# 0411tony/Yue

Measured on AMD Instinct MI355X. Metric: BPR triplet-updates/sec at k=128 (S-round semantics, user rows sequential; the reference's exact sequential semantics: secondary.exact), higher is better.
Workload: dtype f32

## Files before the change

### yue_amd/csrc/bpr_device.hpp

```cpp
#pragma once
#include <hip/hip_runtime.h>
#include <stdint.h>

namespace yue {

constexpr int kNllSlots = 1024;
constexpr int kMaxAttempts = 64;

struct TrainArgs {
    float *P, *Q, *dP, *dQ;
    float *stage;
#ifdef YUE_STAMPS
    unsigned long long *stamps;
#endif
    const int32_t *ev_u, *ev_i;
    int32_t *ev_j;
    const int64_t *indptr;
    const int32_t *indices;
    double *nll_slots;
    int64_t m, n;
    int k;
    float ru, ri;
    double lr;
    uint64_t seed;
    uint32_t epoch;
    int32_t neg_lo, neg_range;
};

struct RoundArgs {
    int64_t e_begin, e_end;
    int64_t n_begin, n_end;
    unsigned long long *cnt_cur;
    unsigned long long *cnt_next;
    uint32_t *cntp_cur;
    uint32_t *cntp_next;
    uint32_t *tab_cur, *tab_next;
    int staged;
    int apply_p;
};

__device__ __forceinline__ uint64_t mix64(uint64_t z) {
    z ^= z >> 30; z *= 0xBF58476D1CE4E5B9ull;
    z ^= z >> 27; z *= 0x94D049BB133111EBull;
    z ^= z >> 31; return z;
}

__device__ __forceinline__ int32_t ctr_draw(uint64_t seed, uint32_t epoch, uint64_t e, uint32_t a, int32_t lo, int32_t n_range) {
    uint64_t z = mix64(seed + 0x9E3779B97F4A7C15ull * (e + 1));
    z = mix64(z ^ (0xD1B54A32D192ED03ull * (uint64_t)(epoch + 1) + 0x8CB92BA72F3D8DD7ull * (uint64_t)a));
    return lo + (int32_t)(((z >> 32) * (uint64_t)(uint32_t)n_range) >> 32);
}

__device__ __forceinline__ bool csr_contains(const int64_t *indptr, const int32_t *indices, int64_t row, int32_t x) {
    int64_t lo = indptr[row], hi = indptr[row + 1];
    while (lo < hi) {
        int64_t mid = (lo + hi) >> 1;
        int32_t v = indices[mid];
        if (v < x) lo = mid + 1; else if (v > x) hi = mid; else return true;
    }
    return false;
}

__device__ __forceinline__ int32_t sample_negative(const TrainArgs &a, int32_t u, int64_t e) {
    for (uint32_t t = 0; t < (uint32_t)kMaxAttempts; ++t) {
        int32_t c = ctr_draw(a.seed, a.epoch, (uint64_t)e, t, a.neg_lo, a.neg_range);
        if (!csr_contains(a.indptr, a.indices, u, c)) return c;
    }
    return -1;
}

__device__ __forceinline__ float rdlane(float v, int l) {
    return __builtin_bit_cast(float, __builtin_amdgcn_readlane(__builtin_bit_cast(int, v), l));
}

template <int CTRL>
__device__ __forceinline__ float dpp_mov(float v) {
    return __builtin_bit_cast(float, __builtin_amdgcn_update_dpp(0, __builtin_bit_cast(int, v), CTRL, 0xF, 0xF, true));
}

__device__ __forceinline__ float wave_sum(float v) {
    v = v + dpp_mov<0xB1>(v);
    v = v + dpp_mov<0x4E>(v);
    v = v + dpp_mov<0x141>(v);
    v = v + dpp_mov<0x140>(v);
    float w = v;
    asm volatile("s_nop 1\n\tv_permlane16_swap_b32 %0, %1\n\ts_nop 1" : "+v"(v), "+v"(w));
    v = v + w;
    return rdlane(v, 0) + rdlane(v, 32);
}

__device__ __forceinline__ double chain_exp(double y) {
    const double n = __builtin_rint(y * 1.4426950408889634074);
    double r = __builtin_fma(-n, 6.93147180369123816490e-01, y);
    r = __builtin_fma(-n, 1.90821492927058770002e-10, r);
    const double r2 = r * r;
    const double a0 = __builtin_fma(r, 1.0, 1.0), a1 = __builtin_fma(r, 1.0 / 6.0, 0.5), a2 = __builtin_fma(r, 1.0 / 120.0, 1.0 / 24.0),
                 a3 = __builtin_fma(r, 1.0 / 5040.0, 1.0 / 720.0), a4 = __builtin_fma(r, 1.0 / 362880.0, 1.0 / 40320.0),
                 a5 = __builtin_fma(r, 1.0 / 39916800.0, 1.0 / 3628800.0), a6 = __builtin_fma(r, 1.0 / 6227020800.0, 1.0 / 479001600.0);
    const double r4 = r2 * r2;
    const double b0 = __builtin_fma(a1, r2, a0), b1 = __builtin_fma(a3, r2, a2), b2 = __builtin_fma(a5, r2, a4);
    const double r8 = r4 * r4;
    const double c0 = __builtin_fma(b1, r4, b0), c1 = __builtin_fma(a6, r4, b2);
    return __builtin_ldexp(__builtin_fma(c1, r8, c0), (int)n);
}
__device__ __forceinline__ double chain_rcp(double d) {
    double y = __builtin_amdgcn_rcp(d);
    double e = __builtin_fma(-d, y, 1.0);
    y = __builtin_fma(e, y, y);
    e = __builtin_fma(-d, y, 1.0);
    y = __builtin_fma(e, y, y);
    e = __builtin_fma(-d, y, 1.0);
    y = __builtin_fma(e, y, y);
    const double r = __builtin_fma(-d, y, 1.0);
    const double y2 = __builtin_bit_cast(double, __builtin_bit_cast(long long, y) + (r > 0.0 ? 1ll : -1ll));
    const double r2 = __builtin_fma(-d, y2, 1.0);
    return __builtin_fabs(r2) < __builtin_fabs(r) ? y2 : y;
}

__device__ __forceinline__ double chain_sigmoid(float x) {
    const double xd = (double)x;
    if (__builtin_fabs(xd) <= 700.0) return chain_rcp(1.0 + chain_exp(-xd));
    return 1.0 / (1.0 + exp(-xd));
}
__device__ __forceinline__ float chain_coef_fast(float x, float lr) {
    return lr * __builtin_amdgcn_rcpf(1.0f + __builtin_amdgcn_exp2f(x * 1.44269502162933349609375f));
}

__device__ __forceinline__ float wave_sum_any(float v) {
    v = v + dpp_mov<0xB1>(v);
    v = v + dpp_mov<0x4E>(v);
    v = v + dpp_mov<0x141>(v);
    v = v + dpp_mov<0x140>(v);
    v = v + __builtin_bit_cast(float, __builtin_amdgcn_update_dpp(0, __builtin_bit_cast(int, v), 0x142, 0xA, 0xF, false));
    v = v + __builtin_bit_cast(float, __builtin_amdgcn_update_dpp(0, __builtin_bit_cast(int, v), 0x143, 0xC, 0xF, false));
    return rdlane(v, 63);
}

struct Elem { float p2, qi2, qj2; };
__device__ __forceinline__ Elem bpr_elem(float p, float qi, float qj, float c, float ru, float ri) {
    const float d = qi - qj;
    const float td = c * d;
    const float p1 = p + td;
    const float tq = c * p1;
    const float qi1 = qi + tq;
    const float qj1 = qj - tq;
    const float rp = ru * p1;
    const float ra = ri * qi1;
    const float rb = ri * qj1;
    Elem o;
    o.p2 = p1 - rp;
    o.qi2 = qi1 - ra;
    o.qj2 = qj1 - rb;
    return o;
}

#define YUE_BLOAD(rs, vo, so) __builtin_bit_cast(float, __builtin_amdgcn_raw_buffer_load_b32((rs), (vo), (so), 0))
// ... 20 lines not shown
```

### yue_amd/csrc/bpr_host.hip

```cpp
#include "host_common.hpp"

#include "train_kernels.hpp"
#include "round_kernels.hpp"

using yue_host::fail;
using yue_host::kr_of;
using yue_host::with_kr;
static_assert(yue::kNllSlots == yue_host::kNllSlotsHost && yue::kHeaderSlack == yue_host::kHeaderSlackHost &&
              yue::kMetaStageMax == (uint32_t)yue_host::kMetaStageMaxHost, "host_common.hpp mirrors these");

namespace {

yue::TrainArgs make_args(yue_ctx *c, double lr, double regU, double regI) {
    yue::TrainArgs a{};
    a.P = c->P.p; a.Q = c->Q.p; a.dP = c->dP.p; a.dQ = c->dQ.p;
    a.stage = c->Q.p ? c->Q.p + (size_t)c->n * c->k : nullptr;
    a.ev_u = c->ev_u.p; a.ev_i = c->ev_i.p; a.ev_j = c->ev_j.p;
    a.indptr = c->indptr.p; a.indices = c->indices.p;
    a.nll_slots = c->scal.p;
    a.m = c->m; a.n = c->n; a.k = c->k;
    a.lr = lr;
    a.ru = (float)(lr * regU);
    a.ri = (float)(lr * regI);
    a.neg_lo = 0; a.neg_range = (int32_t)c->n;
    return a;
}

void launch_level(yue_ctx *c, const yue::TrainArgs &a, int64_t e0, int64_t e1) {
    const int tpw = (int)std::min<int64_t>(64, std::max<int64_t>(1, (e1 - e0) / 4096));
    const int64_t waves = (e1 - e0 + tpw - 1) / tpw;
    const dim3 grid((unsigned)((waves + 3) / 4)), block(256);
    with_kr(c->k, [&](auto kr) { hipLaunchKernelGGL(yue::k_bpr_level<kr()>, grid, block, 0, c->stream, a, e0, e1, tpw); });
}

constexpr int kRoundInstances[][2] = {{1, 8}, {1, 16}, {2, 8}, {4, 4}, {1, 4}, {2, 4}, {1, 2}, {2, 2}};

constexpr int default_round_tpw(int kr, bool meta) { return kr == 4 ? 4 : kr == 2 ? 8 : meta ? 8 : 16; }

template <class F, size_t... I>
bool with_round_instance(int kr, int tpw, F &&f, std::index_sequence<I...>) {
    return ((kr == kRoundInstances[I][0] && tpw == kRoundInstances[I][1] &&
             (f(std::integral_constant<int, kRoundInstances[I][0]>{}, std::integral_constant<int, kRoundInstances[I][1]>{}), true)) || ...);
}
template <class F>
bool with_round_instance(int kr, int tpw, F &&f) {
    return with_round_instance(kr, tpw, f, std::make_index_sequence<sizeof kRoundInstances / sizeof kRoundInstances[0]>{});
}

int tpw_of(const yue_ctx *c, bool meta) { return c->opt_round_tpw ? c->opt_round_tpw : default_round_tpw(kr_of(c->k), meta); }

constexpr int64_t kMetaRangeMax = 37 * 1024;
constexpr int64_t kMetaRangesMax = 12;
constexpr int64_t kRoundGenerationsMax = 6;
constexpr double kRoundEventsPerItemRow = 4.0;

bool meta_bucketed(const yue_ctx *c) { return c->n > kMetaRangeMax * kMetaRangesMax || c->opt_round_bucket; }
bool meta_path_fits(const yue_ctx *c) { return c->opt_round_meta && c->n <= ((int64_t)yue::kBucketRangesMax << yue::kBucketShift); }

// ... 435 lines not shown
    const size_t mk = (size_t)c->m * c->k * sizeof(float), nk = (size_t)c->n * c->k * sizeof(float);
    if (mU) HIPCHK(hipMemcpy(mU, c->aU_m.p, mk, hipMemcpyDeviceToHost));
    if (vU) HIPCHK(hipMemcpy(vU, c->aU_v.p, mk, hipMemcpyDeviceToHost));
    if (mV) HIPCHK(hipMemcpy(mV, c->aV_m.p, nk, hipMemcpyDeviceToHost));
    if (vV) HIPCHK(hipMemcpy(vV, c->aV_v.p, nk, hipMemcpyDeviceToHost));
    return YUE_OK;
}

int yue_adam_step(yue_ctx *c, const int32_t *u, const int32_t *i, const int32_t *j, int64_t T, double lr, double reg, int64_t step, double *loss_out) {
    if (!c || !c->have_factors) return fail(YUE_ERR_ARG, "yue_adam_step: no factors uploaded");
    if (T <= 0 || !u || !i || !j || step < 1) return fail(YUE_ERR_ARG, "yue_adam_step: bad argument (T > 0, step >= 1)");
    HIPCHK(hipSetDevice(c->device));
    if (c->adam_m != c->m || c->adam_n != c->n || c->adam_k != c->k) { const int rc0 = yue_adam_reset(c); if (rc0) return rc0; }
    for (int64_t t = 0; t < T; ++t)
        if (u[t] < 0 || u[t] >= c->m || i[t] < 0 || i[t] >= c->n || j[t] < 0 || j[t] >= c->n) return fail(YUE_ERR_ARG, "yue_adam_step: triplet " + std::to_string(t) + " out of range");
    int rc = upload_triplets(c, u, i, j, T, true);
    if (rc) return rc;
    if ((rc = zero_scalars(c))) return rc;
    yue::MbArgs a{};
    a.U = c->P.p; a.V = c->Q.p; a.gU = c->dP.p; a.gV = c->dQ.p; a.k = c->k; a.u = c->xu.p; a.i = c->xi.p; a.j = c->xj.p; a.T = T;
    a.reg = (float)reg; a.loss_slots = c->scal.p;
    const dim3 grid((unsigned)(((T + 31) / 32 + 3) / 4));
    with_kr(c->k, [&](auto kr) { hipLaunchKernelGGL(yue::k_mb_grad<kr()>, grid, dim3(256), 0, c->stream, a); });
    if ((rc = yue_host::adam_apply(c, lr, step))) return rc;
    return read_scalars(c, loss_out, nullptr, nullptr);
}

int yue_sample_negatives(yue_ctx *c, uint64_t seed, uint32_t epoch, int32_t *j_out) {
    if (!c || !c->have_inter || !j_out) return fail(YUE_ERR_ARG, "yue_sample_negatives: no interactions uploaded");
    HIPCHK(hipSetDevice(c->device));
    yue::TrainArgs a = make_args(c, 0, 0, 0);
    a.seed = seed; a.epoch = epoch;
    if (c->E > 0) {
        hipLaunchKernelGGL(yue::k_sample, dim3((unsigned)((c->E + 255) / 256)), dim3(256), 0, c->stream, a, c->E);
        HIPCHK(hipGetLastError());
        HIPCHK(hipMemcpyAsync(j_out, c->ev_j.p, c->E * sizeof(int32_t), hipMemcpyDeviceToHost, c->stream));
    }
    HIPCHK(hipStreamSynchronize(c->stream));
    return YUE_OK;
}

int yue_sumsq(yue_ctx *c, double *sp, double *sq) {
    if (!c || !c->have_factors) return fail(YUE_ERR_ARG, "yue_sumsq: no factors uploaded");
    HIPCHK(hipSetDevice(c->device));
    int rc = sumsq_async(c);
    if (rc) return rc;
    double h[2];
    HIPCHK(hipMemcpyAsync(h, c->scal.p + yue::kNllSlots + 1, sizeof h, hipMemcpyDeviceToHost, c->stream));
    HIPCHK(hipStreamSynchronize(c->stream));
    if (sp) *sp = h[0];
    if (sq) *sq = h[1];
    return YUE_OK;
}

int yue_bpr_epoch(yue_ctx *c, uint64_t seed, uint32_t epoch, int64_t round_events, double lr, double regU, double regI,
                  double *nll_out, double *sumsqP_out, double *sumsqQ_out) {
    if (!c || !c->have_factors || !c->have_inter) return fail(YUE_ERR_ARG, "yue_bpr_epoch: upload factors and interactions first");
    if (round_events < 0) return fail(YUE_ERR_ARG, "yue_bpr_epoch: round_events must be positive (or 0 for the device's default)");
    HIPCHK(hipSetDevice(c->device));
    yue::TrainArgs a = make_args(c, lr, regU, regI);
    a.seed = seed + 0x632BE59BD9B4E019ull * (uint64_t)c->rank;
    a.epoch = epoch;
    int rc = zero_scalars(c);
    if (rc) return rc;
    const int64_t E = c->E;
    if (E > 0) hipLaunchKernelGGL(yue::k_sample, dim3((unsigned)((E + 255) / 256)), dim3(256), 0, c->stream, a, E);
    if (c->opt_epoch_exact) {
        if (yue_host::on_communicator(c) && c->nranks > 1) return fail(YUE_ERR_ARG, "yue_bpr_epoch: option epoch_exact runs on one GPU (the sequential order spans all item shards)");
        if ((rc = yue_host::chain_epoch(c, lr, regU, regI))) return rc;
        if ((rc = sumsq_async(c))) return rc;
        return read_scalars(c, nll_out, sumsqP_out, sumsqQ_out);
    }
    std::vector<int64_t> bounds;
    double tot[2] = {(double)E, (double)c->n};
    if (yue_host::on_communicator(c)) {
        if ((rc = yue_allreduce_f64(c, tot, 2))) return rc;
        if ((rc = zero_scalars(c))) return rc;
    }
    const double etot = tot[0];
    if (round_events == 0 && (rc = default_round_events(c, tot[1] / c->nranks, &round_events))) return rc;
    int64_t ub = 1, group = 1;
    if ((rc = yue_epoch_plan(c->m, c->k, round_events, etot, c->nranks, &ub, &group, nullptr))) return rc;
    if (!yue_host::on_communicator(c)) group = std::max<int64_t>(1, (c->m + ub - 1) / ub);
    else group = std::max<int64_t>(1, ((int64_t)c->opt_comm_group_mb << 20) / std::max<int64_t>(1, ub * c->k * 4));
    std::vector<int64_t> ublock;
    for (int64_t u0 = 0; u0 < c->m; u0 += ub) { ublock.push_back(u0); bounds.push_back(c->h_ev_ptr[(size_t)u0]); }
    ublock.push_back(c->m); bounds.push_back(E);
    const int64_t R = (int64_t)ublock.size() - 1;
    const bool seq_user = !yue_host::on_communicator(c) && c->opt_round_user_seq && meta_path_fits(c);
    if (seq_user) {
        HIPCHK(c->d_ev_ptr.resize((size_t)c->m + 1));
        if (!c->d_ev_ptr_valid) {
            HIPCHK(hipMemcpyAsync(c->d_ev_ptr.p, c->h_ev_ptr.data(), ((size_t)c->m + 1) * sizeof(int64_t), hipMemcpyHostToDevice, c->stream));
            c->d_ev_ptr_valid = true;
        }
        HIPCHK(c->margins.resize((size_t)std::max<int64_t>(E, 1)));
    }
    c->psq_in_rounds = seq_user && c->all_users_have_events && E > 0;
    if (c->psq_in_rounds) {
        HIPCHK(c->psq_slots.resize((size_t)yue::kNllSlots));
        HIPCHK(hipMemsetAsync(c->psq_slots.p, 0, (size_t)yue::kNllSlots * sizeof(double), c->stream));
    }
    c->last_round_user_seq = 0;
    auto after = [&](int64_t r) -> int {
        if (seq_user && !c->bigq) { c->last_round_user_seq = 1; return YUE_OK; }
        if ((r + 1) % group != 0 && r + 1 != R) return YUE_OK;
        const int64_t g_first = ublock[(size_t)(r - (r % group))], g_last = ublock[(size_t)r + 1];
        const int64_t first = g_first * c->k, count = (g_last - g_first) * c->k;
        const dim3 grid((unsigned)std::min<int64_t>(4096, (count + 255) / 256));
        if (!yue_host::on_communicator(c)) {
            hipLaunchKernelGGL(yue::k_apply_range, grid, dim3(256), 0, c->stream, c->P.p, c->dP.p, first, count);
            return YUE_OK;
        }
        HIPCHK(hipEventRecord(c->ev_rounds, c->stream));
        HIPCHK(hipStreamWaitEvent(c->comm_stream, c->ev_rounds, 0));
        c->comm_collectives += 1;
        c->comm_bytes += (double)count * sizeof(float);
        if (const int rcr = yue_host::reduce_user_block(c, first, count, c->comm_stream)) return rcr;
        hipLaunchKernelGGL(yue::k_apply_range, grid, dim3(256), 0, c->comm_stream, c->P.p, c->dP.p, first, count);
        return YUE_OK;
    };
    c->comm_collectives = 0; c->comm_bytes = 0.0; c->comm_wait_ms = 0.0;
    if ((rc = run_rounds(c, a, bounds, 0, after, meta_path_fits(c), seq_user ? &ublock : nullptr))) { reset_round_state(c); return rc; }
    if (c->last_round_user_seq && E > 0)
        hipLaunchKernelGGL(yue::k_loss_margins, dim3(2048), dim3(256), 0, c->stream, c->margins.p, c->ev_j.p, E, c->scal.p);
    const bool psq_done = c->psq_in_rounds && c->last_round_user_seq;
    c->psq_in_rounds = false;
    if (yue_host::on_communicator(c)) {
        HIPCHK(hipEventRecord(c->ev_t_rounds, c->stream));
        HIPCHK(hipEventRecord(c->ev_t_comm, c->comm_stream));
    }
    HIPCHK(hipEventRecord(c->ev_comm, c->comm_stream));
    HIPCHK(hipStreamWaitEvent(c->stream, c->ev_comm, 0));
    c->comm_compute_waits = 1;
    HIPCHK(hipGetLastError());
    if ((rc = sumsq_async(c, psq_done ? c->psq_slots.p : nullptr))) return rc;
    if ((rc = read_scalars(c, nll_out, sumsqP_out, sumsqQ_out))) return rc;
    if (yue_host::on_communicator(c)) {
        float ms = 0.f;
        HIPCHK(hipEventSynchronize(c->ev_t_comm));
        HIPCHK(hipEventElapsedTime(&ms, c->ev_t_rounds, c->ev_t_comm));
        c->comm_wait_ms = ms > 0.f ? ms : 0.0;
    }
    return YUE_OK;
}

int yue_epoch_plan(int64_t m, int k, int64_t round_events, double events_total, int nranks,
                   int64_t *user_block, int64_t *blocks_per_group, int64_t *n_blocks) {
    if (m <= 0 || k <= 0 || round_events <= 0 || nranks < 1 || !(events_total >= 0.0)) return fail(YUE_ERR_ARG, "yue_epoch_plan: bad argument");
    const double per_user = events_total / (double)nranks / (double)m;
    const int64_t ub = std::max<int64_t>(1, (int64_t)std::floor((double)round_events / std::max(per_user, 1e-9) + 0.5));
    if (user_block) *user_block = ub;
    if (blocks_per_group) *blocks_per_group = std::max<int64_t>(1, (8ll << 20) / std::max<int64_t>(1, ub * k * 4));
    if (n_blocks) *n_blocks = (m + ub - 1) / ub;
    return YUE_OK;
}

int yue_default_round_events(yue_ctx *c, int64_t *out) {
// ... 50 lines not shown
```

### yue_amd/csrc/chain_host.hip

```cpp
#include "host_common.hpp"

#include <rocprim/rocprim.hpp>

#include "chain_kernels.hpp"

using yue_host::fail;
using yue_host::kr_of;

namespace {

int bits_for(uint64_t values) { int b = 1; while ((1ull << b) < values) ++b; return b; }

int rank_in_stream(yue_ctx *c, DevBuf<uint32_t> &key, DevBuf<uint32_t> &val, int64_t count, uint32_t nkeys, uint32_t *ord_a, uint32_t *ord_b) {
    if (count == 0) return YUE_OK;
    HIPCHK(c->ch_key2.resize((size_t)count)); HIPCHK(c->ch_val2.resize((size_t)count)); HIPCHK(c->ch_seg.resize((size_t)nkeys + 1));
    rocprim::double_buffer<uint32_t> dk(key.p, c->ch_key2.p), dv(val.p, c->ch_val2.p);
    size_t tmp = 0;
    const unsigned end_bit = (unsigned)bits_for((uint64_t)nkeys + 1);
    HIPCHK(rocprim::radix_sort_pairs(nullptr, tmp, dk, dv, (size_t)count, 0u, end_bit, c->stream));
    HIPCHK(c->ch_tmp.resize(tmp + 16));
    HIPCHK(rocprim::radix_sort_pairs(c->ch_tmp.p, tmp, dk, dv, (size_t)count, 0u, end_bit, c->stream));
    const dim3 grid((unsigned)((count + 255) / 256));
    hipLaunchKernelGGL(yue::k_chain_seg, grid, dim3(256), 0, c->stream, dk.current(), count, nkeys, c->ch_seg.p);
    hipLaunchKernelGGL(yue::k_chain_ord, grid, dim3(256), 0, c->stream, dk.current(), dv.current(), count, nkeys, c->ch_seg.p, ord_a, ord_b);
// ... 90 lines not shown
    const int64_t blocks = grid.x;
    hipLaunchKernelGGL(yue::k_chain_unpack, dim3(2048), dim3(256), 0, c->stream, c->ch_Qv.p, c->Q.p, n, k);
    if (ord_u) hipLaunchKernelGGL(yue::k_chain_unpack, dim3(2048), dim3(256), 0, c->stream, c->ch_Pv.p, c->P.p, m, k);
    HIPCHK(hipGetLastError());
    unsigned long long ctl[4];
    HIPCHK(hipMemcpyAsync(ctl, c->ch_ctl.p, sizeof ctl, hipMemcpyDeviceToHost, c->stream));
    HIPCHK(hipStreamSynchronize(c->stream));
    const uint32_t st = (uint32_t)ctl[2];
#ifdef YUE_CHAIN_STATS
    {
        unsigned long long h[8];
        HIPCHK(hipMemcpy(h, c->ch_stats.p, sizeof h, hipMemcpyDeviceToHost));
        if (split)
            fprintf(stderr, "[chain3 stats] per triplet: wave C %.0f cycles of work + %.0f waiting for a packet; wave L %.0f cycles per step without a wait (%llu steps) and %.0f waiting for room in the ring; wave S %.0f cycles waiting for packets or answers (%llu triplets)\n",
                    h[1] ? (double)h[0] / h[1] : 0.0, h[1] ? (double)h[2] / h[1] : 0.0, h[4] ? (double)h[3] / h[4] : 0.0, h[4], h[1] ? (double)h[7] / h[1] : 0.0, h[6] ? (double)h[5] / h[6] : 0.0, h[6]);
        else
        fprintf(stderr, "[chain stats] steps without a wait: %llu, %.0f cycles each; steps that waited: %llu (%.2f %%), %.0f cycles each; per run outside the steps: %.0f cycles (%llu runs)\n",
                h[1], h[1] ? (double)h[0] / h[1] : 0.0, h[3], 100.0 * h[3] / (double)(h[1] + h[3] + 1e-9), h[3] ? (double)h[2] / h[3] : 0.0, h[5] ? (double)h[4] / h[5] : 0.0, h[5]);
    }
#endif
    c->chain_runs = R; c->chain_waves = (one_xcd ? c->chain_groups : blocks) * waves_per_block;
    { float ms = 0.0f; HIPCHK(hipEventElapsedTime(&ms, c->ev_chain0, c->ev_chain1)); c->chain_kernel_us = (int64_t)(1e3 * ms); }
    if (st) return fail(YUE_ERR_HIP, std::string("exact path: a wave gave up waiting for a row (") + ((st & 2u) ? "a row's version ran past a waiting touch" : "spin limit") +
                                    "): internal error, the factors on the device are not usable");
    return YUE_OK;
}

}

namespace yue_host {

int chain_epoch(yue_ctx *c, double lr, double regU, double regI) {
    if (c->E == 0) return YUE_OK;
    HIPCHK(c->d_ev_ptr.resize((size_t)c->m + 1));
    if (!c->d_ev_ptr_valid) {
        HIPCHK(hipMemcpyAsync(c->d_ev_ptr.p, c->h_ev_ptr.data(), ((size_t)c->m + 1) * sizeof(int64_t), hipMemcpyHostToDevice, c->stream));
        c->d_ev_ptr_valid = true;
    }
    return chain_launch(c, nullptr, c->ev_i.p, c->ev_j.p, c->E, c->d_ev_ptr.p, nullptr, nullptr, c->m, lr, regU, regI);
}

int chain_stream(yue_ctx *c, int64_t T, double lr, double regU, double regI) {
    if (T == 0) return YUE_OK;
    if (T >= (1ll << 31)) return fail(YUE_ERR_ARG, "exact path: at most 2^31 - 1 triplets per call");
    HIPCHK(c->ch_head.resize((size_t)T)); HIPCHK(c->ch_incl.resize((size_t)T));
    const dim3 tgrid((unsigned)((T + 255) / 256));
    hipLaunchKernelGGL(yue::k_chain_heads, tgrid, dim3(256), 0, c->stream, c->xu.p, T, c->ch_head.p);
    size_t tmp = 0;
    HIPCHK(rocprim::inclusive_scan(nullptr, tmp, c->ch_head.p, c->ch_incl.p, (size_t)T, rocprim::plus<uint32_t>(), c->stream));
    HIPCHK(c->ch_tmp.resize(tmp + 16));
    HIPCHK(rocprim::inclusive_scan(c->ch_tmp.p, tmp, c->ch_head.p, c->ch_incl.p, (size_t)T, rocprim::plus<uint32_t>(), c->stream));
    uint32_t R32 = 0;
    HIPCHK(hipMemcpyAsync(&R32, c->ch_incl.p + (T - 1), sizeof R32, hipMemcpyDeviceToHost, c->stream));
    HIPCHK(hipStreamSynchronize(c->stream));
    const int64_t R = R32;
    HIPCHK(c->ch_run_ptr.resize((size_t)R + 1)); HIPCHK(c->ch_run_u.resize((size_t)R)); HIPCHK(c->ch_ord_u.resize((size_t)R));
    HIPCHK(c->ch_rkey.resize((size_t)R)); HIPCHK(c->ch_rval.resize((size_t)R));
    hipLaunchKernelGGL(yue::k_chain_runs, tgrid, dim3(256), 0, c->stream, c->xu.p, c->ch_head.p, c->ch_incl.p, T, c->ch_run_ptr.p, c->ch_run_u.p, c->ch_rkey.p, c->ch_rval.p, (uint32_t)c->m);
    int rc = rank_in_stream(c, c->ch_rkey, c->ch_rval, R, (uint32_t)c->m, c->ch_ord_u.p, nullptr);
    if (rc) return rc;
    return chain_launch(c, c->xu.p, c->xi.p, c->xj.p, T, c->ch_run_ptr.p, c->ch_run_u.p, c->ch_ord_u.p, R, lr, regU, regI);
}

}
```

### yue_amd/csrc/core_host.hip

```cpp
#include "host_common.hpp"

namespace yue_host {
thread_local std::string g_err;
int fail(int code, const std::string &msg) { g_err = msg; return code; }
}
using yue_host::fail;
void yue_comm_release(yue_ctx *c);

extern "C" {

const char *yue_last_error(void) { return yue_host::g_err.c_str(); }
int yue_version(void) { return 1; }

int yue_ctx_create(int device, yue_ctx **out) {
    if (!out) return fail(YUE_ERR_ARG, "yue_ctx_create: out is NULL");
    int ndev = 0;
    HIPCHK(hipGetDeviceCount(&ndev));
    if (ndev <= 0) return fail(YUE_ERR_HIP, "no HIP device visible: libyue_hip needs an MI355X (no CPU fallback exists)");
    if (device < 0 || device >= ndev) return fail(YUE_ERR_ARG, "device ordinal out of range");
    HIPCHK(hipSetDevice(device));
    yue_ctx *c = new yue_ctx();
    c->device = device;
    const auto init = [c]() -> int {
        HIPCHK(hipStreamCreateWithFlags(&c->stream, hipStreamNonBlocking));
// ... 98 lines not shown
    return YUE_OK;
}

int yue_set_interactions(yue_ctx *c, const int64_t *indptr, const int32_t *indices, const int64_t *ev_ptr, const int32_t *ev_i) {
    if (!c || !indptr || !indices || !ev_ptr || !ev_i) return fail(YUE_ERR_ARG, "yue_set_interactions: null argument");
    if (!c->have_factors) return fail(YUE_ERR_ARG, "yue_set_interactions: call yue_set_factors first (m, n)");
    HIPCHK(hipSetDevice(c->device));
    const int64_t m = c->m, n = c->n;
    if (indptr[0] != 0 || ev_ptr[0] != 0) return fail(YUE_ERR_ARG, "yue_set_interactions: indptr[0] and ev_ptr[0] must be 0");
    for (int64_t u = 0; u < m; ++u) {
        if (indptr[u + 1] < indptr[u] || ev_ptr[u + 1] < ev_ptr[u]) return fail(YUE_ERR_ARG, "yue_set_interactions: offsets must be non-decreasing");
        for (int64_t t = indptr[u]; t < indptr[u + 1]; ++t) {
            if (indices[t] < 0 || indices[t] >= n) return fail(YUE_ERR_ARG, "yue_set_interactions: item id out of range");
            if (t > indptr[u] && indices[t] <= indices[t - 1]) return fail(YUE_ERR_ARG, "yue_set_interactions: rows must be sorted and unique");
        }
        if (indptr[u + 1] - indptr[u] >= n) return fail(YUE_ERR_ARG, "yue_set_interactions: a user listened to every item (the reference's sampler would never return, BPR.py:47)");
    }
    const int64_t nnz = indptr[m], E = ev_ptr[m];
    {
        int64_t prev = -1, max_gap = 0;
        for (int64_t u = 0; u < m; ++u) if (ev_ptr[u + 1] > ev_ptr[u]) { if (prev >= 0) max_gap = std::max(max_gap, u - prev); prev = u; }
        if (max_gap * c->k * 4 >= (1ll << 31)) return fail(YUE_ERR_ARG, "yue_set_interactions: more than 2 GiB of user-factor rows between two consecutive users with events");
    }
    std::vector<int32_t> evu((size_t)E);
    for (int64_t u = 0; u < m; ++u)
        for (int64_t e = ev_ptr[u]; e < ev_ptr[u + 1]; ++e) {
            if (ev_i[e] < 0 || ev_i[e] >= n) return fail(YUE_ERR_ARG, "yue_set_interactions: event item out of range");
            evu[(size_t)e] = (int32_t)u;
        }
    c->E = E; c->nnz = nnz;
    c->h_ev_ptr.assign(ev_ptr, ev_ptr + m + 1);
    c->all_users_have_events = true;
    for (int64_t u = 0; u < m; ++u) if (ev_ptr[u + 1] <= ev_ptr[u]) { c->all_users_have_events = false; break; }
    c->d_ev_ptr_valid = false;
    HIPCHK(c->indptr.resize(m + 1)); HIPCHK(c->indices.resize(std::max<int64_t>(nnz, 1)));
    HIPCHK(c->ev_u.resize((size_t)E + yue_host::kHeaderSlackHost)); HIPCHK(c->ev_i.resize((size_t)E + yue_host::kHeaderSlackHost)); HIPCHK(c->ev_j.resize((size_t)E + yue_host::kHeaderSlackHost));
    HIPCHK(hipMemcpyAsync(c->indptr.p, indptr, (m + 1) * sizeof(int64_t), hipMemcpyHostToDevice, c->stream));
    HIPCHK(hipMemcpyAsync(c->indices.p, indices, nnz * sizeof(int32_t), hipMemcpyHostToDevice, c->stream));
    HIPCHK(hipMemcpyAsync(c->ev_u.p, evu.data(), E * sizeof(int32_t), hipMemcpyHostToDevice, c->stream));
    HIPCHK(hipMemcpyAsync(c->ev_i.p, ev_i, E * sizeof(int32_t), hipMemcpyHostToDevice, c->stream));
    HIPCHK(hipStreamSynchronize(c->stream));
    c->have_inter = true;
    return YUE_OK;
}


}
```

### yue_amd/csrc/host_common.hpp

```cpp
#pragma once
#include "../../include/yue_hip.h"

#include <hip/hip_runtime.h>

#include <algorithm>
#include <cmath>
#include <cstdio>
#include <cstdlib>
#include <cstring>
#include <string>
#include <type_traits>
#include <vector>

struct ncclComm;
struct yue_wrmf;
struct yue_knn;
struct yue_expo;
struct yue_cof;
struct yue_cnet;
struct yue_s2v;
struct yue_lgcn;
struct yue_ipf;

namespace yue_host {
// ... 104 lines not shown
    int opt_round_bucket = 0;
    int opt_fold_blocks = 1536;
    int opt_round_user_seq = 1;
    int opt_round_fast = 1;
    int last_round_user_seq = 0;
    int opt_comm_group_mb = 8;
    int opt_round_cus_reserved = 0;
    int64_t comm_compute_waits = 0;
    int opt_round_meta = 1;
    int timing_stride = 0;
    std::vector<std::pair<hipEvent_t, hipEvent_t>> ev_pool;
    std::vector<int64_t> ev_triplets, ev_launches;
    size_t ev_used = 0;
    DevBuf<double> fP, fBi, f_coef, f_x, f_hist, f_scores, f_out_sc;
    DevBuf<float> fQ;
    DevBuf<int64_t> f_ptr;
    DevBuf<int32_t> f_items, f_negs, f_ids, f_flags;
    DevBuf<int64_t> f_uq_ptr, f_neg_ptr;
    DevBuf<int32_t> f_uq_items, f_loc_i, f_loc_j;
    DevBuf<float> f_wq, f_dQ;
    DevBuf<double> f_wp, f_wb, f_dP, f_dB;
    DevBuf<unsigned> f_cnt;
    int64_t fn = 0;
    int fk = 0;
    int opt_fism_inplace = 1;
    int opt_fism_lds = 1;
    DevBuf<uint32_t> ch_key, ch_val, ch_key2, ch_val2, ch_seg, ch_ord_i, ch_ord_j, ch_head, ch_incl, ch_ord_u, ch_rkey, ch_rval;
    DevBuf<int64_t> ch_run_ptr, d_ev_ptr;
    DevBuf<int32_t> ch_run_u;
    DevBuf<unsigned char> ch_tmp;
    DevBuf<unsigned> ch_Qv, ch_Pv;
    DevBuf<unsigned long long> ch_ctl;
    DevBuf<unsigned long long> ch_stats;
    bool d_ev_ptr_valid = false;
    int opt_epoch_exact = 0;
    int opt_replay_levels = 0;
    int opt_chain_split = -1;
    int opt_chain_ring = 0;
    int opt_chain_xcd = 0;
    int opt_chain_fast = 0;
    int opt_chain_waves = 0;
    int64_t opt_chain_spin = 0;
    int64_t chain_runs = 0, chain_waves = 0, chain_groups = 0, chain_kernel_us = 0, replay_levels = 0;
    hipEvent_t ev_chain0 = nullptr, ev_chain1 = nullptr;
    ncclComm *comm = nullptr;
    int rank = 0, nranks = 1;
    hipStream_t comm_stream = nullptr;
    hipEvent_t ev_rounds = nullptr, ev_comm = nullptr;
    hipEvent_t ev_t_rounds = nullptr, ev_t_comm = nullptr;
    int (*seam_reduce)(void *host, int64_t count, int dtype, void *user) = nullptr;
    void *seam_user = nullptr;
    std::vector<float> seam_buf;
    int64_t comm_collectives = 0;
    double comm_bytes = 0.0, comm_wait_ms = 0.0;
    int comm_version = 0, comm_nranks_reported = 0;
    hipEvent_t ev_scan0 = nullptr, ev_scan1 = nullptr;
    yue_wrmf *wrmf = nullptr;
    yue_knn *knn = nullptr;
    yue_ipf *ipf = nullptr;
    yue_expo *expo = nullptr;
    yue_cof *cof = nullptr;
    yue_cnet *cnet = nullptr;
    yue_s2v *s2v = nullptr;
    yue_lgcn *lgcn = nullptr;
    int64_t opt_lgcn_hub = 1024;
    int64_t lgcn_hubs = 0, lgcn_parts = 0;
    int64_t lgcn_ns[4] = {0, 0, 0, 0};
// ... 45 lines not shown
```

### yue_amd/csrc/round_kernels.hpp

```cpp
#pragma once
#include "train_kernels.hpp"

#ifdef YUE_ABL_NO_HOT
#define YUE_M_HOT(val, rs, vo, so) asm volatile("" :: "v"(val))
#else
#define YUE_M_HOT(val, rs, vo, so) YUE_BATOMIC(val, rs, vo, so)
#endif
#ifdef YUE_ABL_NO_DP
#define YUE_M_DP(val, rs, vo, so) asm volatile("" :: "v"(val))
#else
#define YUE_M_DP(val, rs, vo, so) YUE_BATOMIC(val, rs, vo, so)
#endif

#define YUE_BLOAD_NT(rs, vo, so) __builtin_bit_cast(float, __builtin_amdgcn_raw_buffer_load_b32((rs), (vo), (so), 2))
#if defined(YUE_EXP_LOAD_CACHED)
#define YUE_M_LOAD_J(rs, vo, so) YUE_BLOAD(rs, vo, so)
#define YUE_M_LOAD_I(rs, vo, so) YUE_BLOAD(rs, vo, so)
#elif defined(YUE_EXP_LOAD_NT)
#define YUE_M_LOAD_J(rs, vo, so) YUE_BLOAD_NT(rs, vo, so)
#define YUE_M_LOAD_I(rs, vo, so) YUE_BLOAD_NT(rs, vo, so)
#else
#define YUE_M_LOAD_J(rs, vo, so) YUE_BLOAD_NT(rs, vo, so)
#define YUE_M_LOAD_I(rs, vo, so) YUE_BLOAD(rs, vo, so)
#endif
// ... 399 lines not shown
    const int64_t wave = (int64_t)blockIdx.x * 4 + __builtin_amdgcn_readfirstlane((int)(threadIdx.x >> 6));
    const int64_t u = ra.u_begin + wave;
    if (u >= ra.u_end) return;
    const int64_t e0 = ra.ev_ptr[u], e1 = ra.ev_ptr[u + 1];
    if (e1 <= e0) return;
    const unsigned k = (unsigned)a.k;
    const unsigned row_bytes = k * 4u;
    unsigned vo[KR];
#pragma unroll
    for (int r = 0; r < KR; ++r) { const unsigned e = 64u * r + lane; vo[r] = e < k ? e * 4u : kOobOffset; }
    const uint64_t qbytes = (uint64_t)a.n * row_bytes;
    const int qrec = (int)(qbytes < 0x7fffffffull ? qbytes : 0x7fffffffull);
    const unsigned stage0 = (unsigned)a.n * row_bytes;
    const uint64_t qsbytes = qbytes + (ra.staged ? 2ull * (uint64_t)(ra.e_end - ra.e_begin) * row_bytes : 0ull);
    const int qsrec = (int)(qsbytes < 0x7fffffffull ? qsbytes : 0x7fffffffull);
    const auto rsQ = __builtin_amdgcn_make_buffer_rsrc(a.Q, 0, qsrec, kRsrcFlags);
    const auto rsdQ = __builtin_amdgcn_make_buffer_rsrc(a.dQ, 0, qrec, kRsrcFlags);
    float *prow = a.P + (uint64_t)u * k;
    float p[KR];
#pragma unroll
    for (int r = 0; r < KR; ++r) { const unsigned e = 64u * r + lane; p[r] = e < k ? prow[e] : 0.0f; }
    const float lrf = (float)a.lr;
    const unsigned len = (unsigned)(e1 - e0 < 0x7fffffff ? e1 - e0 : 0x7fffffff);
    for (unsigned seg = 0; seg < len; seg += 64u) {
        int hI, hJ;
        uint32_t hMI, hMJ;
        {
            const bool ex = seg + (unsigned)lane < len;
            const int64_t e = e0 + seg + (ex ? lane : 0);
            hI = evi[e]; hJ = evj[e]; hMI = mti[e]; hMJ = mtj[e];
            if (!ex) { hI = 0; hJ = -1; hMI = 0u; hMJ = 0u; }
        }
        const unsigned seg_len = len - seg < 64u ? len - seg : 64u;
        float xs = 0.0f;
        auto gather = [&](float (&qi)[KR], float (&qj)[KR], unsigned t) {
            const int ti = __builtin_amdgcn_readlane(hI, t), tj = __builtin_amdgcn_readlane(hJ, t);
            const unsigned oi = (unsigned)ti * row_bytes, oj = (unsigned)(tj < 0 ? 0 : tj) * row_bytes;
#pragma unroll
            for (int r = 0; r < KR; ++r) { qi[r] = YUE_M_LOAD_I(rsQ, vo[r], oi); qj[r] = YUE_M_LOAD_J(rsQ, vo[r], oj); }
        };
        auto step = [&](const float (&qi)[KR], const float (&qj)[KR], unsigned t) {
            const int tj = __builtin_amdgcn_readlane(hJ, t);
            if (tj < 0) return;
            const int ti = __builtin_amdgcn_readlane(hI, t);
            const uint32_t mi = (uint32_t)__builtin_amdgcn_readlane((int)hMI, t), mj = (uint32_t)__builtin_amdgcn_readlane((int)hMJ, t);
            float ai = 0.0f, aj = 0.0f;
#pragma unroll
            for (int r = 0; r < KR; ++r) { const float a1 = p[r] * qi[r]; ai = ai + a1; const float a2 = p[r] * qj[r]; aj = aj + a2; }
            const float x = wave_sum(ai) - wave_sum(aj);
            const float c = FAST ? chain_coef_fast(x, lrf) : (float)(a.lr * (1.0 - chain_sigmoid(x)));
            xs = (unsigned)lane == t ? x : xs;
            const unsigned cli = meta_kind(mi), clj = meta_kind(mj);
            const bool uniq_i = cli == kMetaUnique, uniq_j = clj == kMetaUnique;
            const bool full_i = uniq_i || meta_first(mi), full_j = uniq_j || meta_first(mj);
            const unsigned oi = (unsigned)ti * row_bytes, oj = (unsigned)tj * row_bytes;
            const unsigned wi = uniq_i ? oi : stage0 + meta_slot(mi) * row_bytes;
            const unsigned wj = uniq_j ? oj : stage0 + meta_slot(mj) * row_bytes;
            Elem o[KR];
#pragma unroll
            for (int r = 0; r < KR; ++r) { o[r] = bpr_elem(p[r], qi[r], qj[r], c, a.ru, a.ri); p[r] = o[r].p2; }
            if (cli != kMetaHot) {
#pragma unroll
                for (int r = 0; r < KR; ++r) YUE_BSTORE(full_i ? o[r].qi2 : o[r].qi2 - qi[r], rsQ, vo[r], wi);
            } else {
#pragma unroll
                for (int r = 0; r < KR; ++r) YUE_M_HOT(o[r].qi2 - qi[r], rsdQ, vo[r], oi);
            }
            if (clj != kMetaHot) {
#pragma unroll
                for (int r = 0; r < KR; ++r) YUE_BSTORE(full_j ? o[r].qj2 : o[r].qj2 - qj[r], rsQ, vo[r], wj);
            } else {
#pragma unroll
                for (int r = 0; r < KR; ++r) YUE_M_HOT(o[r].qj2 - qj[r], rsdQ, vo[r], oj);
            }
        };
        constexpr int D = KR == 1 ? 8 : 4;
        float qi[D][KR], qj[D][KR];
#pragma unroll
        for (int s_ = 0; s_ < D; ++s_) gather(qi[s_], qj[s_], (unsigned)s_);
        for (unsigned t = 0; t < seg_len; t += D) {
#pragma unroll
            for (int s_ = 0; s_ < D; ++s_) {
                step(qi[s_], qj[s_], t + s_);
                gather(qi[s_], qj[s_], (t + s_ + D) & 63u);
            }
        }
        if ((unsigned)lane < seg_len) ra.margins[e0 + seg + lane] = xs;
    }
#pragma unroll
    for (int r = 0; r < KR; ++r) { const unsigned e = 64u * r + lane; if (e < k) prow[e] = p[r]; }
    if (ra.psq_slots) {
        double s = 0.0;
#pragma unroll
        for (int r = 0; r < KR; ++r) { const unsigned e = 64u * r + lane; const float sq = p[r] * p[r]; if (e < k) s += (double)sq; }
#pragma unroll
        for (int off = 1; off < 64; off <<= 1) s += __shfl_xor(s, off);
        if (lane == 0) atomicAdd(ra.psq_slots + (u & (kNllSlots - 1)), s);
    }
}

__global__ void __launch_bounds__(256) k_loss_margins(const float *__restrict__ x, const int32_t *__restrict__ evj, int64_t E, double *nll_slots) {
    double nl = 0.0;
    const int64_t stride = (int64_t)gridDim.x * blockDim.x;
    for (int64_t e = (int64_t)blockIdx.x * blockDim.x + threadIdx.x; e < E; e += stride)
        if (evj[e] >= 0) nl += -log(chain_sigmoid(x[e]));
#pragma unroll
    for (int off = 1; off < 64; off <<= 1) nl += __shfl_xor(nl, off);
    if ((threadIdx.x & 63) == 0 && nl != 0.0) atomicAdd(nll_slots + ((blockIdx.x * 4 + (threadIdx.x >> 6)) & (kNllSlots - 1)), nl);
}

struct FoldArgs {
    const uint2 *fold;
    const unsigned long long *round_rows;
    float *Q, *dQ;
    const float *stage;
    int k;
    uint32_t capacity;
};

template <int KR, int EPG>
__device__ __forceinline__ void fold_group(const FoldArgs &f, int lane, unsigned k, uint32_t nact, const uint2 (&ent)[4]) {
    float st[EPG][4][KR];
    unsigned el[KR];
    bool big = false;
#pragma unroll
    for (int r = 0; r < KR; ++r) el[r] = min(64u * r + lane, k - 1u);
#pragma unroll
    for (int sl = 0; sl < EPG; ++sl) {
        if ((uint32_t)sl >= nact) continue;
        const uint32_t c = fold_count(ent[sl].y);
        const bool hot = c == 0u;
        const float *src = hot ? f.dQ + (uint64_t)ent[sl].x * k : f.stage + (uint64_t)fold_block(ent[sl].y) * k;
#pragma unroll
        for (int r = 0; r < KR; ++r) st[sl][0][r] = YUE_FOLD_LD(src + el[r]);
        if (hot) {
            const float *row = f.Q + (uint64_t)ent[sl].x * k;
#pragma unroll
            for (int r = 0; r < KR; ++r) st[sl][1][r] = YUE_FOLD_LDROW(row + el[r]);
// ... 95 lines not shown
```

### yue_amd/csrc/train_kernels.hpp

```cpp
#pragma once
#include "bpr_device.hpp"

namespace yue {

__global__ void __launch_bounds__(256) k_sample(TrainArgs a, int64_t E) {
    int64_t e = (int64_t)blockIdx.x * blockDim.x + threadIdx.x;
    if (e < E) a.ev_j[e] = sample_negative(a, a.ev_u[e], e);
}

template <int KR>
__global__ void __launch_bounds__(256) k_bpr_level(TrainArgs a, int64_t e_begin, int64_t e_end, int tpw) {
    const int lane = threadIdx.x & 63;
    const int64_t wave = (int64_t)blockIdx.x * (blockDim.x >> 6) + (threadIdx.x >> 6);
    const int64_t base = e_begin + wave * tpw;
    if (base >= e_end) return;
    const int cnt = (int)((e_end - base) < (int64_t)tpw ? (e_end - base) : (int64_t)tpw);
    int u = 0, i = 0, j = 0;
    if (lane < cnt) { u = a.ev_u[base + lane]; i = a.ev_i[base + lane]; j = a.ev_j[base + lane]; }
    const int k = a.k;
    double nll = 0.0;
    for (int t = 0; t < cnt; ++t) {
        const int64_t tu = __builtin_amdgcn_readlane(u, t);
        const int64_t ti = __builtin_amdgcn_readlane(i, t);
        const int64_t tj = __builtin_amdgcn_readlane(j, t);
        float p[KR], qi[KR], qj[KR];
#pragma unroll
        for (int r = 0; r < KR; ++r) {
            const int e = 64 * r + lane;
            p[r] = e < k ? a.P[tu * k + e] : 0.0f;
            qi[r] = e < k ? a.Q[ti * k + e] : 0.0f;
            qj[r] = e < k ? a.Q[tj * k + e] : 0.0f;
        }
        float ai = 0.0f, aj = 0.0f;
#pragma unroll
        for (int r = 0; r < KR; ++r) { const float a1 = p[r] * qi[r]; ai = ai + a1; const float a2 = p[r] * qj[r]; aj = aj + a2; }
        const float x = wave_sum(ai) - wave_sum(aj);
        const double s = 1.0 / (1.0 + exp(-(double)x));
        const float c = (float)(a.lr * (1.0 - s));
        nll += -log(s);
#pragma unroll
// ... 472 lines not shown
```

Measured before the change: 1.794 billion.

## Sample negatives per user wave with lane-resident rows; vectorize loss kernel

Adds a user-major negative sampler. Each wave owns a user, keeps short CSR rows (up to 64 items) in lanes and tests membership with a ds_bpermute binary search instead of a global-memory binary search per candidate. It prefetches the next user's pointers and row, and falls back to the old per-event kernel when users have few events. The loss kernel now reads margins as float4, takes one log of the product of four sigmoid inverses, and drops the ev_j check by seeding skipped margins with a large sentinel. The ev_ptr upload moves to setup. This trades a small numeric change in the loss sum (product-then-log, sentinel adds a tiny nonzero term) for less memory traffic.

```diff
diff --git a/yue_amd/csrc/bpr_device.hpp b/yue_amd/csrc/bpr_device.hpp
--- a/yue_amd/csrc/bpr_device.hpp
+++ b/yue_amd/csrc/bpr_device.hpp
@@ -45,20 +45,35 @@
     z ^= z >> 31; return z;
 }
 
-__device__ __forceinline__ int32_t ctr_draw(uint64_t seed, uint32_t epoch, uint64_t e, uint32_t a, int32_t lo, int32_t n_range) {
-    uint64_t z = mix64(seed + 0x9E3779B97F4A7C15ull * (e + 1));
-    z = mix64(z ^ (0xD1B54A32D192ED03ull * (uint64_t)(epoch + 1) + 0x8CB92BA72F3D8DD7ull * (uint64_t)a));
+__device__ __forceinline__ uint64_t ctr_draw_event(uint64_t seed, uint64_t e) { return mix64(seed + 0x9E3779B97F4A7C15ull * (e + 1)); }
+__device__ __forceinline__ int32_t ctr_draw_attempt(uint64_t ze, uint32_t epoch, uint32_t a, int32_t lo, int32_t n_range) {
+    const uint64_t z = mix64(ze ^ (0xD1B54A32D192ED03ull * (uint64_t)(epoch + 1) + 0x8CB92BA72F3D8DD7ull * (uint64_t)a));
     return lo + (int32_t)(((z >> 32) * (uint64_t)(uint32_t)n_range) >> 32);
 }
+__device__ __forceinline__ int32_t ctr_draw(uint64_t seed, uint32_t epoch, uint64_t e, uint32_t a, int32_t lo, int32_t n_range) {
+    return ctr_draw_attempt(ctr_draw_event(seed, e), epoch, a, lo, n_range);
+}
 
-__device__ __forceinline__ bool csr_contains(const int64_t *indptr, const int32_t *indices, int64_t row, int32_t x) {
-    int64_t lo = indptr[row], hi = indptr[row + 1];
+__device__ __forceinline__ bool sorted_contains(const int32_t *indices, int64_t lo, int64_t hi, int32_t x) {
     while (lo < hi) {
         int64_t mid = (lo + hi) >> 1;
         int32_t v = indices[mid];
         if (v < x) lo = mid + 1; else if (v > x) hi = mid; else return true;
     }
     return false;
+}
+__device__ __forceinline__ bool csr_contains(const int64_t *indptr, const int32_t *indices, int64_t row, int32_t x) {
+    return sorted_contains(indices, indptr[row], indptr[row + 1], x);
+}
+
+__device__ __forceinline__ bool lanes_contain(int32_t row, int32_t x) {
+    int pos = 0;
+#pragma unroll
+    for (int step = 32; step >= 1; step >>= 1) {
+        const int32_t v = __builtin_amdgcn_ds_bpermute((pos + step - 1) << 2, row);
+        pos += v < x ? step : 0;
+    }
+    return __builtin_amdgcn_ds_bpermute(pos << 2, row) == x;
 }
 
 __device__ __forceinline__ int32_t sample_negative(const TrainArgs &a, int32_t u, int64_t e) {
@@ -122,6 +137,11 @@
     if (__builtin_fabs(xd) <= 700.0) return chain_rcp(1.0 + chain_exp(-xd));
     return 1.0 / (1.0 + exp(-xd));
 }
+__device__ __forceinline__ double chain_inv_sigmoid(float x) {
+    const double xd = (double)x;
+    return 1.0 + (__builtin_fabs(xd) <= 700.0 ? chain_exp(-xd) : exp(-xd));
+}
+constexpr float kMarginNoNegative = 128.0f;
 __device__ __forceinline__ float chain_coef_fast(float x, float lr) {
     return lr * __builtin_amdgcn_rcpf(1.0f + __builtin_amdgcn_exp2f(x * 1.44269502162933349609375f));
 }
diff --git a/yue_amd/csrc/bpr_host.hip b/yue_amd/csrc/bpr_host.hip
--- a/yue_amd/csrc/bpr_host.hip
+++ b/yue_amd/csrc/bpr_host.hip
@@ -24,6 +24,15 @@
     a.ri = (float)(lr * regI);
     a.neg_lo = 0; a.neg_range = (int32_t)c->n;
     return a;
+}
+
+void launch_sample(yue_ctx *c, const yue::TrainArgs &a) {
+    if (c->E >= (int64_t)yue::kSampleWaveEvents * c->m) {
+        const dim3 grid((unsigned)std::min<int64_t>(yue::kSampleBlocksMax, (c->m + 3) / 4));
+        hipLaunchKernelGGL(yue::k_sample, grid, dim3(256), 0, c->stream, a, c->d_ev_ptr.p, c->indptr.p, c->indices.p, c->ev_j.p);
+    } else {
+        hipLaunchKernelGGL(yue::k_sample_events, dim3((unsigned)((c->E + 255) / 256)), dim3(256), 0, c->stream, a, c->E);
+    }
 }
 
 void launch_level(yue_ctx *c, const yue::TrainArgs &a, int64_t e0, int64_t e1) {
@@ -525,7 +534,7 @@
     yue::TrainArgs a = make_args(c, 0, 0, 0);
     a.seed = seed; a.epoch = epoch;
     if (c->E > 0) {
-        hipLaunchKernelGGL(yue::k_sample, dim3((unsigned)((c->E + 255) / 256)), dim3(256), 0, c->stream, a, c->E);
+        launch_sample(c, a);
         HIPCHK(hipGetLastError());
         HIPCHK(hipMemcpyAsync(j_out, c->ev_j.p, c->E * sizeof(int32_t), hipMemcpyDeviceToHost, c->stream));
     }
@@ -557,7 +566,7 @@
     int rc = zero_scalars(c);
     if (rc) return rc;
     const int64_t E = c->E;
-    if (E > 0) hipLaunchKernelGGL(yue::k_sample, dim3((unsigned)((E + 255) / 256)), dim3(256), 0, c->stream, a, E);
+    if (E > 0) launch_sample(c, a);
     if (c->opt_epoch_exact) {
         if (yue_host::on_communicator(c) && c->nranks > 1) return fail(YUE_ERR_ARG, "yue_bpr_epoch: option epoch_exact runs on one GPU (the sequential order spans all item shards)");
         if ((rc = yue_host::chain_epoch(c, lr, regU, regI))) return rc;
@@ -581,14 +590,7 @@
     ublock.push_back(c->m); bounds.push_back(E);
     const int64_t R = (int64_t)ublock.size() - 1;
     const bool seq_user = !yue_host::on_communicator(c) && c->opt_round_user_seq && meta_path_fits(c);
-    if (seq_user) {
-        HIPCHK(c->d_ev_ptr.resize((size_t)c->m + 1));
-        if (!c->d_ev_ptr_valid) {
-            HIPCHK(hipMemcpyAsync(c->d_ev_ptr.p, c->h_ev_ptr.data(), ((size_t)c->m + 1) * sizeof(int64_t), hipMemcpyHostToDevice, c->stream));
-            c->d_ev_ptr_valid = true;
-        }
-        HIPCHK(c->margins.resize((size_t)std::max<int64_t>(E, 1)));
-    }
+    if (seq_user) HIPCHK(c->margins.resize((size_t)std::max<int64_t>(E, 1)));
     c->psq_in_rounds = seq_user && c->all_users_have_events && E > 0;
     if (c->psq_in_rounds) {
         HIPCHK(c->psq_slots.resize((size_t)yue::kNllSlots));
@@ -616,7 +618,7 @@
     c->comm_collectives = 0; c->comm_bytes = 0.0; c->comm_wait_ms = 0.0;
     if ((rc = run_rounds(c, a, bounds, 0, after, meta_path_fits(c), seq_user ? &ublock : nullptr))) { reset_round_state(c); return rc; }
     if (c->last_round_user_seq && E > 0)
-        hipLaunchKernelGGL(yue::k_loss_margins, dim3(2048), dim3(256), 0, c->stream, c->margins.p, c->ev_j.p, E, c->scal.p);
+        hipLaunchKernelGGL(yue::k_loss_margins, dim3(2048), dim3(256), 0, c->stream, c->margins.p, E, c->scal.p);
     const bool psq_done = c->psq_in_rounds && c->last_round_user_seq;
     c->psq_in_rounds = false;
     if (yue_host::on_communicator(c)) {
diff --git a/yue_amd/csrc/chain_host.hip b/yue_amd/csrc/chain_host.hip
--- a/yue_amd/csrc/chain_host.hip
+++ b/yue_amd/csrc/chain_host.hip
@@ -146,11 +146,6 @@
 
 int chain_epoch(yue_ctx *c, double lr, double regU, double regI) {
     if (c->E == 0) return YUE_OK;
-    HIPCHK(c->d_ev_ptr.resize((size_t)c->m + 1));
-    if (!c->d_ev_ptr_valid) {
-        HIPCHK(hipMemcpyAsync(c->d_ev_ptr.p, c->h_ev_ptr.data(), ((size_t)c->m + 1) * sizeof(int64_t), hipMemcpyHostToDevice, c->stream));
-        c->d_ev_ptr_valid = true;
-    }
     return chain_launch(c, nullptr, c->ev_i.p, c->ev_j.p, c->E, c->d_ev_ptr.p, nullptr, nullptr, c->m, lr, regU, regI);
 }
 
diff --git a/yue_amd/csrc/core_host.hip b/yue_amd/csrc/core_host.hip
--- a/yue_amd/csrc/core_host.hip
+++ b/yue_amd/csrc/core_host.hip
@@ -154,11 +154,11 @@
     c->h_ev_ptr.assign(ev_ptr, ev_ptr + m + 1);
     c->all_users_have_events = true;
     for (int64_t u = 0; u < m; ++u) if (ev_ptr[u + 1] <= ev_ptr[u]) { c->all_users_have_events = false; break; }
-    c->d_ev_ptr_valid = false;
-    HIPCHK(c->indptr.resize(m + 1)); HIPCHK(c->indices.resize(std::max<int64_t>(nnz, 1)));
+    HIPCHK(c->indptr.resize(m + 1)); HIPCHK(c->indices.resize(std::max<int64_t>(nnz, 1))); HIPCHK(c->d_ev_ptr.resize((size_t)m + 1));
     HIPCHK(c->ev_u.resize((size_t)E + yue_host::kHeaderSlackHost)); HIPCHK(c->ev_i.resize((size_t)E + yue_host::kHeaderSlackHost)); HIPCHK(c->ev_j.resize((size_t)E + yue_host::kHeaderSlackHost));
     HIPCHK(hipMemcpyAsync(c->indptr.p, indptr, (m + 1) * sizeof(int64_t), hipMemcpyHostToDevice, c->stream));
     HIPCHK(hipMemcpyAsync(c->indices.p, indices, nnz * sizeof(int32_t), hipMemcpyHostToDevice, c->stream));
+    HIPCHK(hipMemcpyAsync(c->d_ev_ptr.p, ev_ptr, (m + 1) * sizeof(int64_t), hipMemcpyHostToDevice, c->stream));
     HIPCHK(hipMemcpyAsync(c->ev_u.p, evu.data(), E * sizeof(int32_t), hipMemcpyHostToDevice, c->stream));
     HIPCHK(hipMemcpyAsync(c->ev_i.p, ev_i, E * sizeof(int32_t), hipMemcpyHostToDevice, c->stream));
     HIPCHK(hipStreamSynchronize(c->stream));
diff --git a/yue_amd/csrc/host_common.hpp b/yue_amd/csrc/host_common.hpp
--- a/yue_amd/csrc/host_common.hpp
+++ b/yue_amd/csrc/host_common.hpp
@@ -160,7 +160,6 @@
     DevBuf<unsigned> ch_Qv, ch_Pv;
     DevBuf<unsigned long long> ch_ctl;
     DevBuf<unsigned long long> ch_stats;
-    bool d_ev_ptr_valid = false;
     int opt_epoch_exact = 0;
     int opt_replay_levels = 0;
     int opt_chain_split = -1;
diff --git a/yue_amd/csrc/round_kernels.hpp b/yue_amd/csrc/round_kernels.hpp
--- a/yue_amd/csrc/round_kernels.hpp
+++ b/yue_amd/csrc/round_kernels.hpp
@@ -455,7 +455,7 @@
             if (!ex) { hI = 0; hJ = -1; hMI = 0u; hMJ = 0u; }
         }
         const unsigned seg_len = len - seg < 64u ? len - seg : 64u;
-        float xs = 0.0f;
+        float xs = kMarginNoNegative;
         auto gather = [&](float (&qi)[KR], float (&qj)[KR], unsigned t) {
             const int ti = __builtin_amdgcn_readlane(hI, t), tj = __builtin_amdgcn_readlane(hJ, t);
             const unsigned oi = (unsigned)ti * row_bytes, oj = (unsigned)(tj < 0 ? 0 : tj) * row_bytes;
@@ -522,11 +522,24 @@
     }
 }
 
-__global__ void __launch_bounds__(256) k_loss_margins(const float *__restrict__ x, const int32_t *__restrict__ evj, int64_t E, double *nll_slots) {
+__device__ __forceinline__ double loss_of_four(const float4 x) {
+    const double d0 = chain_inv_sigmoid(x.x), d1 = chain_inv_sigmoid(x.y), d2 = chain_inv_sigmoid(x.z), d3 = chain_inv_sigmoid(x.w);
+    if (fminf(fminf(x.x, x.y), fminf(x.z, x.w)) > -170.0f) return log((d0 * d1) * (d2 * d3));
+    return (log(d0) + log(d1)) + (log(d2) + log(d3));
+}
+__global__ void __launch_bounds__(256) k_loss_margins(const float *__restrict__ x, int64_t E, double *nll_slots) {
     double nl = 0.0;
-    const int64_t stride = (int64_t)gridDim.x * blockDim.x;
-    for (int64_t e = (int64_t)blockIdx.x * blockDim.x + threadIdx.x; e < E; e += stride)
-        if (evj[e] >= 0) nl += -log(chain_sigmoid(x[e]));
+    const int64_t stride = (int64_t)gridDim.x * blockDim.x, G = E >> 2;
+    const float4 *x4 = reinterpret_cast<const float4 *>(x);
+    int64_t g = (int64_t)blockIdx.x * blockDim.x + threadIdx.x;
+    for (; g + stride < G; g += 2 * stride) {
+        const float4 a = x4[g], b = x4[g + stride];
+        nl += loss_of_four(a);
+        nl += loss_of_four(b);
+    }
+    if (g < G) nl += loss_of_four(x4[g]);
+    const int64_t e = 4 * G + (int64_t)blockIdx.x * blockDim.x + threadIdx.x;
+    if (e < E) nl += log(chain_inv_sigmoid(x[e]));
 #pragma unroll
     for (int off = 1; off < 64; off <<= 1) nl += __shfl_xor(nl, off);
     if ((threadIdx.x & 63) == 0 && nl != 0.0) atomicAdd(nll_slots + ((blockIdx.x * 4 + (threadIdx.x >> 6)) & (kNllSlots - 1)), nl);
diff --git a/yue_amd/csrc/train_kernels.hpp b/yue_amd/csrc/train_kernels.hpp
--- a/yue_amd/csrc/train_kernels.hpp
+++ b/yue_amd/csrc/train_kernels.hpp
@@ -3,9 +3,47 @@
 
 namespace yue {
 
-__global__ void __launch_bounds__(256) k_sample(TrainArgs a, int64_t E) {
+__global__ void __launch_bounds__(256) k_sample_events(TrainArgs a, int64_t E) {
     int64_t e = (int64_t)blockIdx.x * blockDim.x + threadIdx.x;
     if (e < E) a.ev_j[e] = sample_negative(a, a.ev_u[e], e);
+}
+
+constexpr int kSampleBlocksMax = 2048;
+constexpr int kSampleWaveEvents = 32;
+__global__ void __launch_bounds__(256) k_sample(TrainArgs a, const int64_t *__restrict__ ev_ptr, const int64_t *__restrict__ indptr,
+                                                const int32_t *__restrict__ indices, int32_t *__restrict__ ev_j) {
+    const int lane = threadIdx.x & 63;
+    const int64_t stride = (int64_t)gridDim.x * 4;
+    int64_t u = (int64_t)blockIdx.x * 4 + __builtin_amdgcn_readfirstlane((int)(threadIdx.x >> 6));
+    struct User { int64_t e0, e1, r0, r1; };
+    auto pointers = [&](int64_t v) {
+        User s{0, 0, 0, 0};
+        if (v < a.m) { s.e0 = ev_ptr[v]; s.e1 = ev_ptr[v + 1]; s.r0 = indptr[v]; s.r1 = indptr[v + 1]; }
+        return s;
+    };
+    auto row_of = [&](const User &s) { return s.r1 - s.r0 <= 64 && s.r0 + lane < s.r1 ? indices[s.r0 + lane] : INT32_MAX; };
+    User cur = pointers(u), nxt = pointers(u + stride);
+    int32_t row = row_of(cur);
+    for (; u < a.m; u += stride) {
+        const int32_t row_nxt = row_of(nxt);
+        const User after = pointers(u + 2 * stride);
+        const bool in_lanes = cur.r1 - cur.r0 <= 64;
+        for (int64_t eb = cur.e0; eb < cur.e1; eb += 64) {
+            const int64_t e = eb + lane;
+            const uint64_t ze = ctr_draw_event(a.seed, (uint64_t)e);
+            bool pending = e < cur.e1;
+            int32_t neg = -1;
+            for (uint32_t t = 0; t < (uint32_t)kMaxAttempts && __builtin_amdgcn_ballot_w64(pending) != 0; ++t) {
+                const int32_t c = ctr_draw_attempt(ze, a.epoch, t, a.neg_lo, a.neg_range);
+                bool hit;
+                if (in_lanes) hit = lanes_contain(row, c);
+                else hit = pending && sorted_contains(indices, cur.r0, cur.r1, c);
+                if (pending && !hit) { neg = c; pending = false; }
+            }
+            if (e < cur.e1) ev_j[e] = neg;
+        }
+        cur = nxt; nxt = after; row = row_nxt;
+    }
 }
 
 template <int KR>
```

Result: faster. 1.820 billion (median of 6 runs) (+1.4%).
